# sloisel/MultiGridBarrier.jl

Hardware: AMD Instinct MI355X
Metric: Newton iters/sec + wall-clock to converge, 2D P2 p-Laplace L=9 (higher is better)
Workload: dtype f64

## Files before the change

include/mgbhip.h:

```cpp
#ifndef MGBHIP_H
#define MGBHIP_H

#include <stdint.h>

#ifdef __cplusplus
extern "C" {
#endif

#define MGBHIP_OK 0
#define MGBHIP_ERR_INVALID 1
#define MGBHIP_ERR_HIP 2
#define MGBHIP_ERR_NOT_SPD 3
#define MGBHIP_ERR_NONFINITE 4
#define MGBHIP_ERR_CONVERGENCE 5

#define MGBHIP_MAX_PIECES 4
#define MGBHIP_MAX_IDX 10
#define MGBHIP_MAX_LIN 4
#define MGBHIP_MAX_ND 13
#define MGBHIP_MAX_NU 4
#define MGBHIP_MAX_OPS 8

#define MGBHIP_KIND_EP 1
#define MGBHIP_KIND_LINEAR 2
// ... 116 lines not shown

int mgbhip_mgb_core(mgbhip_problem* prob, double* z , const double* c ,
                    const mgbhip_options* opt, mgbhip_core_result* res);
int mgbhip_matched_t(mgbhip_problem* prob, const double* z, const double* c, double t_default,
                     double* t_out);
void mgbhip_default_options(mgbhip_options* opt, int64_t n_nodes);

typedef struct mgbhip_vec mgbhip_vec;
int mgbhip_vec_alloc(mgbhip_ctx* ctx, int64_t len, mgbhip_vec** out);
int mgbhip_vec_free(mgbhip_vec* v);
int64_t mgbhip_vec_len(const mgbhip_vec* v);
int mgbhip_vec_upload(mgbhip_vec* v, const double* host, int64_t len);
int mgbhip_vec_download(const mgbhip_vec* v, double* host, int64_t len);
int mgbhip_vec_fill(mgbhip_vec* v, double value);
int mgbhip_vec_copy(mgbhip_vec* dst, const mgbhip_vec* src);
int mgbhip_vec_axpy(double alpha, const mgbhip_vec* x, mgbhip_vec* y);
int mgbhip_vec_scale(double alpha, mgbhip_vec* x);
int mgbhip_vec_dot(const mgbhip_vec* a, const mgbhip_vec* b, double* out);
int mgbhip_vec_norm(const mgbhip_vec* a, double* out);
int mgbhip_vec_isfinite(const mgbhip_vec* a, int32_t* all_finite);
int mgbhip_f0_d(mgbhip_problem* prob, int32_t level, const mgbhip_vec* s, const mgbhip_vec* c,
                const mgbhip_vec* z0, double* value);
int mgbhip_f1_d(mgbhip_problem* prob, int32_t level, const mgbhip_vec* s, const mgbhip_vec* c,
                const mgbhip_vec* z0, mgbhip_vec* grad);
int mgbhip_f2_d(mgbhip_problem* prob, int32_t level, const mgbhip_vec* s, const mgbhip_vec* c,
                const mgbhip_vec* z0);
int mgbhip_solve_d(mgbhip_problem* prob, int32_t level, const mgbhip_vec* g, mgbhip_vec* x);
int mgbhip_prolong_add(mgbhip_problem* prob, int32_t level, const mgbhip_vec* s, mgbhip_vec* z);

int mgbhip_stage_ms(mgbhip_problem* prob, const char* stage, double* total_ms, int64_t* launches);
int mgbhip_reset_stage_timers(mgbhip_problem* prob, int enable);
int mgbhip_solver_stats(mgbhip_problem* prob, int32_t level, double* out8);
int mgbhip_solver_chain(mgbhip_problem* prob, int32_t level, double* out8);
enum { MGBHIP_PROJ_NONE = 0, MGBHIP_PROJ_LOOP = 1, MGBHIP_PROJ_STAGED = 2, MGBHIP_PROJ_MFMA = 3, MGBHIP_PROJ_ACCUMULATE = 4 };
int mgbhip_level_plan(mgbhip_problem* prob, int32_t level, int32_t* out16);

#define MGBHIP_INTERP_FEM1D 1
#define MGBHIP_INTERP_QK 2
#define MGBHIP_INTERP_P1 3
#define MGBHIP_INTERP_P2 4
#define MGBHIP_INTERP_SPECTRAL1D 5
#define MGBHIP_INTERP_SPECTRAL2D 6
int mgbhip_interpolate(mgbhip_ctx* ctx, int32_t family, int32_t d, int32_t k, int32_t p, int64_t N,
                       const double* x, const double* table, int32_t ncomp, const double* z, int64_t M,
                       const double* pts, double* out, int32_t* elem);
int mgbhip_interpolate_grad(mgbhip_ctx* ctx, int32_t family, int32_t d, int32_t k, int32_t p, int64_t N,
                            const double* x, const double* table, int32_t ncomp, const double* z, int64_t M,
                            const double* pts, double* out ,
                            double* grad , int32_t* elem );

typedef struct mgbhip_locator mgbhip_locator;
int mgbhip_locator_create(mgbhip_ctx* ctx, int32_t family, int32_t d, int32_t k, int32_t p, int64_t N,
                          const double* x, const double* table, int64_t M, const double* pts,
                          mgbhip_locator** out);
int mgbhip_locator_elements(const mgbhip_locator* loc, int32_t* elem );
int mgbhip_locator_evaluate(mgbhip_locator* loc, int32_t ncomp, const double* z ,
                            double* out ,
                            double* grad );
int mgbhip_locator_destroy(mgbhip_locator* loc);

typedef struct mgbhip_contour mgbhip_contour;
int mgbhip_contour_create(mgbhip_ctx* ctx, int32_t family, int32_t d, int32_t k, int32_t p, int64_t N,
                          const double* x, const double* table, int32_t nfield , const double* fields,
                          int32_t nlevels, const double* levels, int32_t refine,
                          mgbhip_contour** out, int64_t* nsimplices);
int mgbhip_contour_fetch(const mgbhip_contour* c, double* points, int32_t* level, int32_t* element,
                         double* carried );
// ... 35 lines not shown
```

multigridbarrier.jl_amd/csrc/kernels.hip:

```cpp
#include <hip/hip_runtime.h>

#include <algorithm>
#include <mutex>

#include "kernels.hpp"
#include "dense.hpp"

namespace mgbhip {

namespace {

template <int CTRL>
__device__ __forceinline__ double dpp_mov_f64(double v) {
    const long long b = __double_as_longlong(v);
    const int lo = __builtin_amdgcn_mov_dpp((int)(b & 0xffffffffll), CTRL, 0xF, 0xF, true);
    const int hi = __builtin_amdgcn_mov_dpp((int)(b >> 32), CTRL, 0xF, 0xF, true);
    return __longlong_as_double(((long long)hi << 32) | (unsigned int)lo);
}
__device__ __forceinline__ double z_at(const ElemParams& P, int64_t i) {
    double v = P.z0[i];
    if (P.zsel) {
        const int32_t c = P.zsel[i];
        if (c >= 0) v += P.zx ? __builtin_fma(-P.zalpha, P.zx[c], P.zs[c]) : P.zs[c];
        if (P.zout) P.zout[i] = v;
// ... 419 lines not shown
                                } else if (idk) {
                                    val += Yt[i] * OP(k2, i, j);
                                } else if (idk2) {
                                    val += OP(k, j, i) * Yt[j];
                                } else {
                                    double acc = 0.0;
                                    for (int rr = 0; rr < p; ++rr) acc += OP(k, rr, i) * Yt[rr] * OP(k2, rr, j);
                                    val += acc;
                                }
                            }
                        }
                        out[i] = val;
                    }
                }
        }
        return;
    }
}

struct SigRuntime {
    static constexpr bool rt = true;
    static __device__ __forceinline__ constexpr int state(int) { return 0; }
    static __device__ __forceinline__ constexpr int stage(int) { return 0; }
    static __device__ __forceinline__ constexpr int mask() { return 0; }
};
template <int NY>
struct SigDefault {
    static constexpr bool rt = false;
    static __device__ __forceinline__ constexpr int state(int k) { return k == NY - 1 ? 1 : 0; }
    static __device__ __forceinline__ constexpr int stage(int k) { return (k == 0 || k == NY - 1) ? -1 : k - 1; }
    static __device__ __forceinline__ constexpr int mask() { return ((1 << NY) - 1) & ~1; }
};

template <int NY, int P, class Sig, bool CONDENSE = false>
__global__ __launch_bounds__(256) void elem_f2_fast(const ElemParams Pm) {
    constexpr int G = (P <= 2) ? 2 : (P <= 4) ? 4 : (P <= 8) ? 8 : (P <= 16) ? 16 : (P <= 32) ? 32 : 64;
    constexpr int EPB = 256 / G;
    constexpr int PP = P * P;
    constexpr int NT = NY * (NY + 1) / 2;
    extern __shared__ double sh[];
    const int tid = threadIdx.x;
    const int el = tid / G;
    const int r = tid % G;
    const int nu = Sig::rt ? Pm.nu : 2;
    auto DST = [&](int k) -> int { return Sig::rt ? Pm.D_state[k] : Sig::state(k); };
    auto DSG = [&](int k) -> int { return Sig::rt ? Pm.D_stage[k] : Sig::stage(k); };
    const int ymask = Sig::rt ? Pm.ymask : Sig::mask();
    const int64_t e0 = (int64_t)blockIdx.x * EPB;
    const int64_t e = e0 + el;
    const bool active = (e < Pm.N) && (r < P);
    const int64_t n = Pm.n;
    const int64_t node = e * P + r;

    double* zl = sh;
    double* opL = zl + 256 * nu;
    double* YL = opL + (size_t)Pm.nstage * EPB * PP;

    double zr[MGBHIP_MAX_NU];
#pragma unroll
    for (int a = 0; a < MGBHIP_MAX_NU; ++a) zr[a] = (active && a < nu) ? z_at(Pm, (int64_t)a * n + node) : 0.0;
    {
        int64_t lim = (Pm.N - e0) * PP;
        if (lim > (int64_t)EPB * PP) lim = (int64_t)EPB * PP;
        constexpr int NIT = (EPB * PP + 255) / 256;
        for (int o = 0; o < Pm.nstage; ++o) {
            const double* src = Pm.stage_ptr[o] + e0 * PP;
            double* dst = opL + (size_t)o * EPB * PP;
// ... 20 lines not shown
    auto OP = [&](int k, int rr, int cc) -> double { return opE[(size_t)DSG(k) * EPB * PP + cc * P + rr]; };

    double y[NY];
#pragma unroll
    for (int k = 0; k < NY; ++k) {
        double v = 0.0;
        if (active) {
            const double* za = zl + (el * nu + DST(k)) * G;
            if (DSG(k) < 0) v = za[r];
            else {
#pragma unroll
                for (int cc = 0; cc < P; ++cc) v += OP(k, r, cc) * za[cc];
            }
        }
        y[k] = v;
    }
    if (active) {
        double F, g[NY], H[NY * NY];
        cone_eval<NY, 2>(Pm.cone, node, n, y, F, g, H);
        const double bwv = Pm.bw ? Pm.bw[node] : 0.0;
#pragma unroll
        for (int k = 0; k < NY; ++k)
#pragma unroll
            for (int k2 = k; k2 < NY; ++k2) {
                const double h = H[k * NY + k2];
                YL[((size_t)el * NT + (k * NY - (k * (k - 1)) / 2 + (k2 - k))) * G + r] =
                    Pm.bw ? ((bwv == 0.0) ? 0.0 : bwv * h) : Pm.invn * h;
            }
    }
    __syncthreads();
    const int j = r;
    const double* Ye = YL + (size_t)el * NT * G;
    int blk = 0;
    double cblk[CONDENSE ? 3 : 1][P];
#pragma unroll
    for (int a = 0; a < nu; ++a)
#pragma unroll
        for (int b = a; b < nu; ++b, ++blk) {
            const bool dblk = CONDENSE ? (blk == 2) : ((Pm.diag_mask >> blk) & 1);
            double* dst = CONDENSE ? &cblk[blk < 3 ? blk : 0][0]
                                   : Pm.out_hel + Pm.blk_off[blk] + (dblk ? (e * P + j) : (e * P + j) * (int64_t)P);
            bool b_all_id = true;
#pragma unroll
            for (int k2 = 0; k2 < NY; ++k2)
                if (DST(k2) == b && ((ymask >> k2) & 1) && DSG(k2) >= 0) b_all_id = false;
            if (active && b_all_id) {
                double Cd[NY];
#pragma unroll
                for (int k = 0; k < NY; ++k) {
                    double acc = 0.0;
                    if (DST(k) == a && ((ymask >> k) & 1)) {
#pragma unroll
                        for (int k2 = 0; k2 < NY; ++k2) {
                            if (DST(k2) != b || !((ymask >> k2) & 1)) continue;
                            const int t = (k <= k2) ? (k * NY - (k * (k - 1)) / 2 + (k2 - k))
                                                    : (k2 * NY - (k2 * (k2 - 1)) / 2 + (k - k2));
                            acc += Ye[t * G + j];
                        }
                    }
                    Cd[k] = acc;
                }
                if (dblk) {
                    double val = 0.0;
#pragma unroll
                    for (int k = 0; k < NY; ++k)
                        if (DST(k) == a && ((ymask >> k) & 1)) val += Cd[k];
                    dst[0] = val;
                } else {
#pragma unroll
                    for (int i = 0; i < P; ++i) {
                        double val = 0.0;
#pragma unroll
                        for (int k = 0; k < NY; ++k) {
// ... 129 lines not shown
                    if (rr > j) S[at(rr, j)] = 0.0;
                S[at(P, j)] = usc[PB] * inv;
#pragma unroll
                for (int i = 0; i < PB; ++i)
                    if (pos[i] != 15) S[at(pos[i], j)] = usc[i] * inv;
                S[at(m - 1, j)] = beta * inv;
                if (j == PB) {
                    S[at(P, P)] = d7;
#pragma unroll
                    for (int i = 0; i < PB; ++i)
                        if (pos[i] != 15) S[at(pos[i], P)] = xc[i] * inv7;
                    S[at(m - 1, P)] = bb * inv7;
                    S[at(m - 1, m - 1)] = corner - bb * bb * inv7;
                } else if (pos[j] != 15) {
#pragma unroll
                    for (int i = 0; i < PB; ++i)
                        if (pos[i] != 15 && pos[i] >= pos[j]) S[at(pos[i], pos[j])] = up[i] - xc[i] * f;
                    S[at(m - 1, pos[j])] = bj - bb * f;
                }
            }
            if (pk) {
                __builtin_amdgcn_fence(__ATOMIC_RELEASE, "wavefront");
                __builtin_amdgcn_wave_barrier();
                __builtin_amdgcn_fence(__ATOMIC_ACQUIRE, "wavefront");
                if (e < Pm.N) {
                    const LeafDesc l2 = Pm.leaf_desc[e];
                    const int mm = (int)(l2.packed & 15u);
                    double* dstF = Pm.leaf_arena + l2.F_off;
                    for (int t = r; t < mm * (mm + 1) / 2; t += G) dstF[t] = S[t];
                }
            }
        }
        if (bad) atomicOr(Pm.leaf_status, 1);
    }
}

template <int NY, int P, class Sig>
__global__ __launch_bounds__(256) void elem_f01_fast(const ElemParams Pm) {
    constexpr int G = (P <= 2) ? 2 : (P <= 4) ? 4 : (P <= 8) ? 8 : (P <= 16) ? 16 : (P <= 32) ? 32 : 64;
    constexpr int EPB = 256 / G;
    constexpr int PP = P * P;
    extern __shared__ double sh[];
    const int tid = threadIdx.x;
    const int el = tid / G;
    const int r = tid % G;
    const int nu = Sig::rt ? Pm.nu : 2;
    auto DST = [&](int k) -> int { return Sig::rt ? Pm.D_state[k] : Sig::state(k); };
    auto DSG = [&](int k) -> int { return Sig::rt ? Pm.D_stage[k] : Sig::stage(k); };
    const int64_t e0 = (int64_t)blockIdx.x * EPB;
    const int64_t e = e0 + el;
    const bool active = (e < Pm.N) && (r < P);
    const int64_t n = Pm.n;
    const int64_t node = e * P + r;

    double* zl = sh;
    double* opL = zl + 256 * nu;
    double* YL = opL + (size_t)Pm.nstage * EPB * PP;
    {
        int64_t lim = (Pm.N - e0) * PP;
        if (lim > (int64_t)EPB * PP) lim = (int64_t)EPB * PP;
        constexpr int NIT = (EPB * PP + 255) / 256;
        for (int o = 0; o < Pm.nstage; ++o) {
            const double* src = Pm.stage_ptr[o] + e0 * PP;
            double* dst = opL + (size_t)o * EPB * PP;
            double v[NIT];
#pragma unroll
// ... 924 lines not shown
        (void)hipFuncSetAttribute((const void*)elem_f2_fast<NY, PN, SigDefault<NY>>, hipFuncAttributeMaxDynamicSharedMemorySize, 160 * 1024);
        (void)hipGetLastError();
        return true;
    }();
    (void)attr;
    if (is_default_signature<NY>(P))
        hipLaunchKernelGGL((elem_f2_fast<NY, PN, SigDefault<NY>>), dim3((unsigned)elem_grid(PN, P.N)), dim3(256), lds, st, P);
    else
        hipLaunchKernelGGL((elem_f2_fast<NY, PN, SigRuntime>), dim3((unsigned)elem_grid(PN, P.N)), dim3(256), lds, st, P);
    return true;
}

bool launch_elem_f2_condense(const ElemParams& P, hipStream_t st) {
    constexpr int NY = 4, PN = 7;
    if (P.wide || P.nD != NY || P.p != PN || P.nu != 2 || P.nstage != 2 || !is_default_signature<NY>(P)) return false;
    for (int k = 0; k < NY; ++k)
        if (P.D_stage[k] == -2) return false;
    MGB_REQUIRE(P.leaf_desc && P.leaf_arena && P.leaf_g && P.leaf_status, "condensing f2: leaf arguments missing");
    const int G = elem_group(PN);
    const int EPB = 256 / G;
    const size_t lds = (256 * (size_t)P.nu + (size_t)P.nstage * EPB * PN * PN + (size_t)EPB * (NY * (NY + 1) / 2) * G) * sizeof(double);
    static bool attr = [] {
        (void)hipFuncSetAttribute((const void*)elem_f2_fast<NY, PN, SigDefault<NY>, true>, hipFuncAttributeMaxDynamicSharedMemorySize, 160 * 1024);
        (void)hipGetLastError();
        return true;
    }();
    (void)attr;
    hipLaunchKernelGGL((elem_f2_fast<NY, PN, SigDefault<NY>, true>), dim3((unsigned)elem_grid(PN, P.N)), dim3(256), lds, st, P);
    MGB_HIP_CHECK(hipGetLastError());
    return true;
}

template <int NY, int PN>
static bool try_f01_fast(const ElemParams& P, hipStream_t st) {
    if (P.nD != NY || P.p != PN) return false;
    for (int k = 0; k < NY; ++k)
        if (P.D_stage[k] == -2) return false;
    const int G = elem_group(PN);
    const int EPB = 256 / G;
    size_t lds = (256 * (size_t)P.nu + (size_t)P.nstage * EPB * PN * PN + (size_t)EPB * NY * G) * sizeof(double);
    if (lds < 256 * sizeof(double)) lds = 256 * sizeof(double);
    if (lds > 160 * 1024) return false;
    static bool attr = [] {
        (void)hipFuncSetAttribute((const void*)elem_f01_fast<NY, PN, SigRuntime>, hipFuncAttributeMaxDynamicSharedMemorySize, 160 * 1024);
        (void)hipFuncSetAttribute((const void*)elem_f01_fast<NY, PN, SigDefault<NY>>, hipFuncAttributeMaxDynamicSharedMemorySize, 160 * 1024);
        (void)hipGetLastError();
        return true;
    }();
    (void)attr;
    if (is_default_signature<NY>(P))
        hipLaunchKernelGGL((elem_f01_fast<NY, PN, SigDefault<NY>>), dim3((unsigned)elem_grid(PN, P.N)), dim3(256), lds, st, P);
    else
        hipLaunchKernelGGL((elem_f01_fast<NY, PN, SigRuntime>), dim3((unsigned)elem_grid(PN, P.N)), dim3(256), lds, st, P);
    return true;
}

size_t wide_lds_bytes(int p, int nu, int nD, int nstage, int mode) {
    const int G = elem_group(p);
    const int threads = (mode == MODE_F2) ? WIDE_F2_THREADS : 256;
    const int EPB = threads / G;
    size_t d = (size_t)threads * nu + (size_t)nstage * EPB * p * p;
    if (mode == MODE_F1 || mode == MODE_F01) d += (size_t)threads * nD;
    if (mode == MODE_F2) d += (size_t)threads * (nD * (nD + 1) / 2);
    if (d < 256) d = 256;
    return d * sizeof(double);
}
// ... 326 lines not shown
void launch_panel_accumulate(const PanelParams& P, const int32_t* ecols, int32_t m, int32_t nstream, int32_t nsplit,
                             int32_t chunk, int32_t ctmax, double* partial, double* H, hipStream_t st) {
    if (m == 0) return;
    const size_t lds = ((size_t)chunk + panel_stage_doubles(P.p, P.nu, ctmax)) * sizeof(double);
    MGB_REQUIRE(lds <= PANEL_ACC_LDS_MAX, "coarse-level accumulator + panels exceed the LDS budget");
    MGB_REQUIRE(panel_accumulate_fits(P.p, P.nu, ctmax), "coarse-level panels exceed the register staging of the accumulation kernel");
    static std::once_flag once;
    std::call_once(once, [] {
        (void)hipFuncSetAttribute((const void*)panel_accumulate_kernel, hipFuncAttributeMaxDynamicSharedMemorySize,
                                  (int)PANEL_ACC_LDS_MAX);
        (void)hipGetLastError();
    });
    hipLaunchKernelGGL(panel_accumulate_kernel, dim3((unsigned)nstream, (unsigned)nsplit), dim3(256), lds, st, P, ecols, m,
                       ctmax, chunk, partial);
    hipLaunchKernelGGL(accumulate_reduce_kernel, dim3((unsigned)(((int64_t)m * m + 255) / 256)), dim3(256), 0, st, m,
                       nstream, partial, H);
    MGB_HIP_CHECK(hipGetLastError());
}

void launch_panel_project_staged(const PanelParams& P, int32_t ctmax, hipStream_t st) {
    if (P.N == 0) return;
    const size_t lds = panel_accumulate_lds(P.p, P.nu, ctmax);
    MGB_REQUIRE(lds <= PANEL_ACC_LDS_MAX, "coarse-level panels too wide for the staged projection kernel");
    static std::once_flag once;
    std::call_once(once, [] {
        (void)hipFuncSetAttribute((const void*)panel_project_staged_kernel, hipFuncAttributeMaxDynamicSharedMemorySize,
                                  (int)PANEL_ACC_LDS_MAX);
        (void)hipGetLastError();
    });
    hipLaunchKernelGGL(panel_project_staged_kernel, dim3((unsigned)((P.N + 3) / 4)), dim3(256), lds, st, P, ctmax);
    MGB_HIP_CHECK(hipGetLastError());
}

bool launch_panel_project_mfma(const PanelParams& P, hipStream_t st) {
    if (P.N == 0) return true;
    if (P.nu > MGBHIP_MAX_NU || P.p > 64) return false;
    const int ctpad = P.nu * pp_round_up(P.cmax, 16);
    const PanelMfmaLayout Y = panel_mfma_layout(P.p, P.nu, ctpad);
    const size_t lds = (size_t)Y.total * sizeof(double);
    static const bool off = [] { const char* e = getenv("MGBHIP_NO_MFMA_PROJECT"); return e && e[0] == '1'; }();
    if (off || lds > 64 * 1024 || ctpad < 48) return false;
    static std::once_flag once;
    std::call_once(once, [] {
        (void)hipFuncSetAttribute((const void*)panel_project_mfma_kernel, hipFuncAttributeMaxDynamicSharedMemorySize, 64 * 1024);
        (void)hipGetLastError();
    });
    hipLaunchKernelGGL(panel_project_mfma_kernel, dim3((unsigned)P.N), dim3(256), lds, st, P, ctpad);
    MGB_HIP_CHECK(hipGetLastError());
    return true;
}

void launch_invert_lists(const int32_t* cidx, int64_t total, int32_t* spos, hipStream_t st) {
    if (total <= 0) return;
    hipLaunchKernelGGL(invert_lists_kernel, dim3((unsigned)((total + 255) / 256)), dim3(256), 0, st, cidx, total, spos);
    MGB_HIP_CHECK(hipGetLastError());
}

void launch_panel_project(const PanelParams& P, hipStream_t st) {
    if (P.N == 0) return;
    const size_t lds = (size_t)4 * P.p * P.cmax * sizeof(double);
    static const bool big_lds = hipFuncSetAttribute((const void*)panel_project_kernel,
                                                    hipFuncAttributeMaxDynamicSharedMemorySize, 144 * 1024) == hipSuccess;
    if (!big_lds) (void)hipGetLastError();
    MGB_REQUIRE(lds <= (big_lds ? 144 : 64) * 1024, "coarse-level panels too wide for the projection kernel");
    hipLaunchKernelGGL(panel_project_kernel, dim3((unsigned)((P.N + 3) / 4)), dim3(256), lds, st, P);
    MGB_HIP_CHECK(hipGetLastError());
}

}
```

multigridbarrier.jl_amd/csrc/kernels.hpp:

```cpp
#pragma once
#include "common.hpp"
#include "cone.hpp"

namespace mgbhip {

enum ElemMode { MODE_F0 = 0, MODE_F1 = 1, MODE_F2 = 2, MODE_NODE_F = 3, MODE_NODE_SLACK = 4,
                MODE_F01 = 5 };

struct LeafDesc {
    int64_t F_off;
    int32_t interior;
    uint32_t packed;
};

struct ElemParams {
    int32_t p, nu, nD, nstage;
    int32_t ymask;
    int64_t N, n;
    const double* ops[MGBHIP_MAX_OPS];
    const double* stage_ptr[MGBHIP_MAX_OPS];
    int32_t D_state[MGBHIP_MAX_ND];
    int32_t D_op[MGBHIP_MAX_ND];
    int32_t D_stage[MGBHIP_MAX_ND];
    const double* w;
    const double* c;
    const double* z0;
    const double* bw;
    double invn;
    ConeDev cone;
    double* out_partial;
    double* out_ret;
    double* out_hel;
    double* out_F;
    double* out_Dz;
    int32_t diag_mask;
    int64_t blk_off[MGBHIP_MAX_NU * (MGBHIP_MAX_NU + 1) / 2];
    double* dn_Dz;
    double* dn_Y;
    const LeafDesc* leaf_desc;
    double* leaf_arena;
    const double* leaf_g;
    int64_t leaf_slack0;
    int32_t* leaf_status;
    int32_t leaf_packed;
    const int32_t* zsel;
    const double* zs;
    double* zout;
    const double* zx;
    double zalpha;
    int32_t wide;
};
static_assert(sizeof(ElemParams) <= 4096 - 64, "ElemParams must stay well inside the kernel argument limit");

bool launch_elem_f2_condense(const ElemParams& P, hipStream_t st);

inline int hel_blocks(int nu) { return nu * (nu + 1) / 2; }
inline int hel_block_index(int a, int b, int nu) { return a * nu - a * (a - 1) / 2 + (b - a); }
inline int64_t hel_layout(int nu, int64_t N, int p, int diag_mask, int64_t* off) {
    int64_t total = 0;
    for (int blk = 0; blk < hel_blocks(nu); ++blk) {
        off[blk] = total;
        total += ((diag_mask >> blk) & 1) ? N * p : N * (int64_t)p * p;
    }
    return total;
}

int elem_group(int p);
constexpr int WIDE_F2_THREADS = 128;
size_t wide_lds_bytes(int p, int nu, int nD, int nstage, int mode);
int64_t elem_grid(int p, int64_t N);
size_t elem_lds_bytes(const ElemParams& P, int mode);
void launch_elem(const ElemParams& P, int mode, hipStream_t st);

void launch_reduce_partials(const double* partials, int64_t count, double* out, hipStream_t st);
void launch_vec_stats(const double* v, int64_t n, double* scratch, double* stats, hipStream_t st, const double* mask = nullptr,
                      const int32_t* ints = nullptr, int nints = 0);
void launch_dir_stats(const double* v, const double* g, int64_t n, double* scratch, double* stats3, hipStream_t st,
                      const double* mask = nullptr, const int32_t* ints = nullptr, int nints = 0);
void launch_dot(const double* a, const double* b, int64_t n, double* scratch, double* out, hipStream_t st, const double* mask = nullptr);
void launch_restrict_trial(int64_t rows, const int32_t* ptr, const int32_t* col, const double* val, const double* ret, double* g,
                            double* scratch, const double* x, const double* nn, double s, double* xn, int32_t* moved, int32_t stamp,
                            hipStream_t st);
void launch_publish(const double* src, int n, double* host_block, int host_lo, double seq, hipStream_t st);
void launch_dir_finish(const double* v, const double* g, int64_t n, double* scratch, double* scal, int32_t* status2, double* host,
                       hipStream_t st, const double* mask = nullptr, double seq = 0.0);
void launch_trial_finish(const double* g, int64_t n, double* scratch, const double* f0_partials, int64_t f0_count, double* scal,
                         int32_t* moved, double* host, hipStream_t st, const double* mask = nullptr, double seq = 0.0,
// ... 5 lines not shown
void launch_csr_matvec(int64_t rows, const int32_t* ptr, const int32_t* col, const double* val,
                       const double* x, double* y, bool add, bool long_rows, hipStream_t st);
int csr_chunks(int64_t max_row_len);
void launch_csr_matvec_chunked(int64_t rows, const int32_t* ptr, const int32_t* col, const double* val,
                               const double* x, double* y, double* scratch, int nchunk, hipStream_t st);
void launch_prolong(int64_t rows, const int32_t* ptr, const int32_t* col, const double* val, const double* s,
                    const double* z0, double* zfull, hipStream_t st);
void launch_step(const double* x, const double* n, double s, double* xn, int64_t len, int32_t* moved, int32_t stamp,
                 hipStream_t st);
void launch_scale_copy(const double* src, double alpha, double* dst, int64_t len, hipStream_t st);
void launch_border_tail(const double* g, double* tail, int64_t m, hipStream_t st);
void launch_axpy(double alpha, const double* x, double* y, int64_t len, hipStream_t st);
void launch_fill(double value, double* y, int64_t len, hipStream_t st);

void launch_gather_shared(int64_t nshared, const int32_t* sh_q, const int32_t* cptr, const int32_t* cidx, const double* slab,
                          double* out, hipStream_t st);
void launch_gather_assemble(int64_t nnz, const int32_t* cptr, const int32_t* cidx, const double* slab,
                            double* Hval, bool long_lists, hipStream_t st, int32_t chunk = 0, int32_t nchunk = 0,
                            double* part = nullptr, const int32_t* qmap = nullptr, int64_t nq = 0);

struct PanelParams {
    int32_t p, nu;
    int64_t N;
    const int32_t* ecol_ptr;
    const double* panels;
    const int32_t* eoff;
    const double* hel;
    double* slab;
    int32_t cmax;
    int32_t upper_only;
    const int32_t* spos;
};
bool launch_panel_project_mfma(const PanelParams& P, hipStream_t st);
void launch_invert_lists(const int32_t* cidx, int64_t total, int32_t* spos, hipStream_t st);
void launch_panel_project(const PanelParams& P, hipStream_t st);
constexpr size_t PANEL_ACC_LDS_MAX = 144 * 1024;
size_t panel_accumulate_lds(int p, int nu, int ctmax);
size_t panel_stage_doubles(int p, int nu, int ctmax);
bool panel_accumulate_fits(int p, int nu, int ctmax);
void launch_panel_accumulate(const PanelParams& P, const int32_t* ecols, int32_t m, int32_t nstream, int32_t nsplit,
                             int32_t chunk, int32_t ctmax, double* partial, double* H, hipStream_t st);
void launch_panel_project_staged(const PanelParams& P, int32_t ctmax, hipStream_t st);

}
```

multigridbarrier.jl_amd/csrc/problem.cpp:

```cpp
#include "problem.hpp"
#include "plan_device.hpp"
#include "dense.hpp"

#include <algorithm>
#include <chrono>
#include <cmath>
#include <cstdio>
#include <atomic>
#include <exception>
#include <cstdlib>
#include <string>
#include <thread>
#include <cstring>
#include <numeric>

using namespace mgbhip;

static constexpr int64_t ACC_MAX_M = 384;



static void upload_csr(const mgbhip_csr& R, Level& L, hipStream_t st) {
    MGB_REQUIRE(R.rows >= 0 && R.cols >= 0 && R.rowptr && (R.rowptr[R.rows] == 0 || (R.colidx && R.values)),
                "bad prolongation CSR");
// ... 813 lines not shown
}

void mgbhip_problem::eval_f2(int level, const double* d_s, const double* d_zz, const double* d_cc, bool materialize,
                             const double* rhs) {
    ensure_plan(level);
    hipStream_t st = stream();
    Level& L = levels[level];
    int E_ymask = 0;
    if (L.condense && !materialize && rhs != nullptr && L.selection && L.direct && !dense) {
        StageScope sc(ctx->timers, level + 1 == (int)levels.size() ? "f2" : "f2_coarse");
        ElemParams E = base_params(level, d_s, d_zz, d_cc);
        E.leaf_desc = L.solver.leaf_desc();
        E.leaf_arena = L.solver.arena();
        E.leaf_g = rhs;
        E.leaf_slack0 = L.m - n;
        E.leaf_status = L.solver.leaf_status();
        E.leaf_packed = L.solver.leaves_packed() ? 1 : 0;
        if (!L.solver.leaf_flag_zero()) MGB_HIP_CHECK(hipMemsetAsync(E.leaf_status, 0, sizeof(int32_t), st));
        L.solver.leaf_flag_used();
        if (launch_elem_f2_condense(E, st)) {
            L.have_H = true;
            L.H_in_slab = true;
            L.H_condensed = true;
            L.condensed_rhs = rhs;
            hel_level = level;
            L.factored = false;
            cnt.f2++;
            return;
        }
        zf_stamp = -1;
    }
    L.H_condensed = false;
    L.proj_kernel = MGBHIP_PROJ_NONE;
    {
        StageScope sc(ctx->timers, level + 1 == (int)levels.size() ? "f2" : "f2_coarse");
        ElemParams E = base_params(level, d_s, d_zz, d_cc);
        E_ymask = E.ymask;
        E.diag_mask = (L.selection && !dense) ? diag_mask_sel : 0;
        hel_layout(nu, N, p, E.diag_mask, E.blk_off);
        launch_elem(E, MODE_F2, st);
    }
    {
        StageScope sc(ctx->timers, level + 1 == (int)levels.size() ? "assemble" : "assemble_coarse");
        if (dense) {
            int klo = nD, khi = -1;
            for (int k = 0; k < nD; ++k)
                if ((E_ymask >> k) & 1) { klo = std::min(klo, k); khi = std::max(khi, k); }
            const int64_t ld = (int64_t)nD * n;
            if (khi < klo) {
                MGB_HIP_CHECK(hipMemsetAsync(L.Hval.p, 0, sizeof(double) * (size_t)L.nnz, st));
            } else {
                launch_dense_weight(nD, klo, khi, n, L.m, ld, L.denseDR.p, d_dnY.p, L.denseW.p, st);
                launch_dense_gemm_tn((int)L.m, (int)L.m, (int)((khi - klo + 1) * n), L.denseDR.p + (int64_t)klo * n, ld,
                                     nullptr, L.denseW.p + (int64_t)klo * n, ld, L.Hval.p, L.m, false, true, st);
            }
        } else if (L.selection && L.direct && !materialize) {
            launch_gather_shared(L.nshared, L.sh_q.p, L.cptr.p, L.cidx.p, d_hel.p, d_hel.p + hel_cap, st);
        } else if (L.selection) {
            launch_gather_assemble(L.nnz, L.cptr.p, L.cidx.p, d_hel.p, L.Hval.p, L.long_lists, st, L.gather_chunk, L.gather_nchunk, L.gather_part.p);
        } else {
            PanelParams PP;
            PP.p = p; PP.nu = nu; PP.N = N;
            PP.ecol_ptr = L.ecol_ptr.p; PP.panels = L.panels.p; PP.eoff = L.eoff.p;
            PP.hel = d_hel.p; PP.slab = L.slab.p; PP.cmax = L.cmax; PP.spos = nullptr;
            static const bool full_h = [] { const char* e = getenv("MGBHIP_FULL_COARSE_H"); return e && e[0] == '1'; }();
            const bool upper = !materialize && rhs != nullptr && L.nup > 0 && !L.acc && !full_h;
            PP.upper_only = upper ? 1 : 0;
            if (L.acc) {
                L.proj_kernel = MGBHIP_PROJ_ACCUMULATE;
                launch_panel_accumulate(PP, L.ecols.p, (int32_t)L.m, L.acc_waves, L.acc_split, L.acc_chunk, L.acc_ctmax,
                                        L.acc_copies.p, L.Hval.p, st);
            } else {
                PP.spos = L.sorted_slab ? L.spos.p : nullptr;
                if (launch_panel_project_mfma(PP, st)) {
                    L.proj_kernel = MGBHIP_PROJ_MFMA;
                } else if (panel_accumulate_lds(p, nu, L.acc_ctmax) <= 40 * 1024) {
                    L.proj_kernel = MGBHIP_PROJ_STAGED;
                    launch_panel_project_staged(PP, L.acc_ctmax, st);
                } else {
                    L.proj_kernel = MGBHIP_PROJ_LOOP;
                    launch_panel_project(PP, st);
                }
                launch_gather_assemble(L.nnz, L.cptr.p, L.sorted_slab ? nullptr : L.cidx.p, L.slab.p, L.Hval.p, L.long_lists, st, L.gather_chunk,
                                       L.gather_nchunk, L.gather_part.p, upper ? L.upq.p : nullptr, upper ? L.nup : 0);
            }
        }
    }
    L.have_H = true;
    L.H_in_slab = L.selection && L.direct && !materialize && !dense;
    hel_level = L.H_in_slab ? level : -1;
    L.factored = false;
    cnt.f2++;
}

void mgbhip_problem::wait_results(double seq) {
    static const bool poll = [] { const char* e = getenv("MGBHIP_NO_POLL"); return !(e && e[0] == '1'); }();
    hipStream_t st = stream();
    if (poll && seq != 0.0) {
        volatile const double* stamp = pin.d + 15;
        const auto t0 = std::chrono::steady_clock::now();
        for (int spins = 0;; ++spins) {
            if (__atomic_load_n(reinterpret_cast<const volatile uint64_t*>(stamp), __ATOMIC_ACQUIRE) ==
                *reinterpret_cast<const uint64_t*>(&seq))
                return;
            if ((spins & 1023) == 1023 &&
                std::chrono::duration<double>(std::chrono::steady_clock::now() - t0).count() > 1e-3)
                break;
// ... 175 lines not shown
```

multigridbarrier.jl_amd/device.py:

```python
from __future__ import annotations

import ctypes as C
import os
import weakref
from typing import List, Optional

import numpy as np
import scipy.sparse as sp

from .blockmatrices import BlockColumn, BlockDiag
from .convex import KIND_EP, KIND_LINEAR, Convex
from .multigrid import AMG
from .problem import MGBProblem

MAX_PIECES, MAX_IDX, MAX_ND, MAX_NU, MAX_OPS = 4, 10, 13, 4, 8
MAX_LIN = 4
OK, ERR_INVALID, ERR_HIP, ERR_NOT_SPD, ERR_NONFINITE, ERR_CONVERGENCE = range(6)


class Device:
    """reference: src/device.jl:18"""


class CPUDevice(Device):
# ... 556 lines not shown
                    factorizations=int(r.factorizations), failure_code=int(r.failure_code), k=int(r.k))
        return status, z, diag

    def matched_t(self, z, c, t_default: float) -> float:
        z = _f64(z)
        c = np.asfortranarray(c, dtype=np.float64)
        out = C.c_double()
        _check(self.lib, self.lib.mgbhip_matched_t(self.handle, _ptr(z), _ptr(c), float(t_default), C.cast(C.byref(out), _dp)))
        return out.value

    def reset_stage_timers(self, enable: bool = True):
        _check(self.lib, self.lib.mgbhip_reset_stage_timers(self.handle, 1 if enable else 0))

    def stage_ms(self, stage: str):
        ms, cnt = C.c_double(), C.c_int64()
        _check(self.lib, self.lib.mgbhip_stage_ms(self.handle, stage.encode(), C.cast(C.byref(ms), _dp), C.byref(cnt)))
        return ms.value, cnt.value

    def solver_stats(self, level: int) -> dict:
        out = np.zeros(8)
        _check(self.lib, self.lib.mgbhip_solver_stats(self.handle, level, _ptr(out)))
        keys = ("fronts", "max_front", "arena_doubles", "factor_flops", "peeled", "tree_levels", "nnz", "unknowns")
        return dict(zip(keys, out.tolist()))

    def solver_chain(self, level: int) -> dict:
        out = np.zeros(8)
        _check(self.lib, self.lib.mgbhip_solver_chain(self.handle, level, _ptr(out)))
        keys = ("pivot_blocks_on_critical_path", "large_front_tree_levels", "launches_per_factorization",
                "launches_per_backward_sweep", "arena_doubles", "factor_flops", "extra_trailing_doubles", "reserved")
        return dict(zip(keys, out.tolist()))

    PLAN_KEYS = ("R_unit", "R_long", "T_long", "T_chunks", "selection", "acc", "acc_split", "long_lists", "gather_chunk",
                 "gather_nchunk", "projection", "max_row", "max_col", "cmax", "mean_list", "planned")
    PROJECTION = ("none", "loop", "staged", "mfma", "accumulate")

    def level_plan(self, level: int) -> dict:
        out = (C.c_int32 * 16)()
        _check(self.lib, self.lib.mgbhip_level_plan(self.handle, level, out))
        d = dict(zip(self.PLAN_KEYS, (int(v) for v in out)))
        d["projection"] = self.PROJECTION[d["projection"]]
        d["direct"] = bool(d["selection"] & 2)
        d["selection"] = bool(d["selection"] & 1)
        for k in ("R_unit", "R_long", "T_long", "acc", "long_lists", "planned"):
            d[k] = bool(d[k])
        return d

    def close(self):
        if self.handle:
            self.lib.mgbhip_problem_destroy(self.handle)
            self.handle = None

    def __del__(self):
        try:
            self.close()
        except Exception:
            pass


def dense_as_block(M: AMG) -> AMG:
    if isinstance(M.D_fine[0], BlockColumn):
        return M
    n = M.w.size
    geom = M.geometry
    ops = {k: BlockDiag(np.asarray(v, dtype=np.float64).reshape(n, n, 1)) for k, v in geom.operators.items()}
    from dataclasses import replace
    g2 = replace(geom, operators=ops)
    nu = len(M.state_names)
# ... 49 lines not shown
```

Before: 674.3.

## Fuse coarse-level panel projection into the element Hessian f2 kernel

Adds a PROJECT variant of elem_f2_fast that keeps each element's 2x2-block Hessian in LDS and immediately projects it through the prolongation panels (P^T H P), writing directly into the coarse slab. It is used when the MFMA projection does not apply, in place of a separate f2 kernel plus a staged projection kernel. This removes the global write and read of the per-element Hessian and one launch per coarse level. In exchange it adds LDS pressure and wave-level serial work per element inside the f2 kernel, and it only covers a few hardcoded (NY,P) instantiations.

```diff
diff --git a/include/mgbhip.h b/include/mgbhip.h
--- a/include/mgbhip.h
+++ b/include/mgbhip.h
@@ -172,7 +172,8 @@
 int mgbhip_reset_stage_timers(mgbhip_problem* prob, int enable);
 int mgbhip_solver_stats(mgbhip_problem* prob, int32_t level, double* out8);
 int mgbhip_solver_chain(mgbhip_problem* prob, int32_t level, double* out8);
-enum { MGBHIP_PROJ_NONE = 0, MGBHIP_PROJ_LOOP = 1, MGBHIP_PROJ_STAGED = 2, MGBHIP_PROJ_MFMA = 3, MGBHIP_PROJ_ACCUMULATE = 4 };
+enum { MGBHIP_PROJ_NONE = 0, MGBHIP_PROJ_LOOP = 1, MGBHIP_PROJ_STAGED = 2, MGBHIP_PROJ_MFMA = 3, MGBHIP_PROJ_ACCUMULATE = 4,
+       MGBHIP_PROJ_FUSED = 5  };
 int mgbhip_level_plan(mgbhip_problem* prob, int32_t level, int32_t* out16);
 
 #define MGBHIP_INTERP_FEM1D 1
diff --git a/multigridbarrier.jl_amd/csrc/kernels.hip b/multigridbarrier.jl_amd/csrc/kernels.hip
--- a/multigridbarrier.jl_amd/csrc/kernels.hip
+++ b/multigridbarrier.jl_amd/csrc/kernels.hip
@@ -475,7 +475,7 @@
     static __device__ __forceinline__ constexpr int mask() { return ((1 << NY) - 1) & ~1; }
 };
 
-template <int NY, int P, class Sig, bool CONDENSE = false>
+template <int NY, int P, class Sig, bool CONDENSE = false, bool PROJECT = false>
 __global__ __launch_bounds__(256) void elem_f2_fast(const ElemParams Pm) {
     constexpr int G = (P <= 2) ? 2 : (P <= 4) ? 4 : (P <= 8) ? 8 : (P <= 16) ? 16 : (P <= 32) ? 32 : 64;
     constexpr int EPB = 256 / G;
@@ -562,13 +562,13 @@
     const int j = r;
     const double* Ye = YL + (size_t)el * NT * G;
     int blk = 0;
-    double cblk[CONDENSE ? 3 : 1][P];
+    double cblk[(CONDENSE || PROJECT) ? 3 : 1][P];
 #pragma unroll
     for (int a = 0; a < nu; ++a)
 #pragma unroll
         for (int b = a; b < nu; ++b, ++blk) {
-            const bool dblk = CONDENSE ? (blk == 2) : ((Pm.diag_mask >> blk) & 1);
-            double* dst = CONDENSE ? &cblk[blk < 3 ? blk : 0][0]
+            const bool dblk = CONDENSE ? (blk == 2) : PROJECT ? false : ((Pm.diag_mask >> blk) & 1);
+            double* dst = (CONDENSE || PROJECT) ? &cblk[blk < 3 ? blk : 0][0]
                                    : Pm.out_hel + Pm.blk_off[blk] + (dblk ? (e * P + j) : (e * P + j) * (int64_t)P);
             bool b_all_id = true;
 #pragma unroll
@@ -764,6 +764,96 @@
             }
         }
         if (bad) atomicOr(Pm.leaf_status, 1);
+    }
+    if constexpr (PROJECT) {
+        static_assert(!Sig::rt && !CONDENSE && P <= 8, "projection: default two-state signature only");
+        constexpr int NBLK = 3, EPW = 64 / G, NROW = 2 * P, NPF = ELEM_PROJECT_PREFETCH;
+        const int lane = tid & 63;
+        const int wave = __builtin_amdgcn_readfirstlane(tid >> 6);
+        const int ctmax = Pm.pj_ctmax;
+        __syncthreads();
+        if (active) {
+            double* Hc = sh + (size_t)el * (NBLK * PP) + P * j;
+#pragma unroll
+            for (int b3 = 0; b3 < NBLK; ++b3)
+#pragma unroll
+                for (int i = 0; i < P; ++i) Hc[b3 * PP + i] = cblk[b3][i];
+        }
+        double* Pl = sh + (size_t)EPB * (NBLK * PP) + (size_t)wave * (3 * P) * ctmax;
+        double* Tl = Pl + (size_t)P * ctmax;
+        int32_t nct = 0, nc0 = 0, neo = 0;
+        double rP[NPF];
+        auto prefetch = [&](int64_t ee) {
+            const int32_t base = Pm.pj_ecol_ptr[ee * 2];
+            nc0 = Pm.pj_ecol_ptr[ee * 2 + 1] - base;
+            nct = Pm.pj_ecol_ptr[ee * 2 + 2] - base;
+            neo = Pm.pj_eoff[ee];
+            const double* pan = Pm.pj_panels + (int64_t)P * base;
+#pragma unroll
+            for (int u = 0; u < NPF; ++u) {
+                const int t = lane + 64 * u;
+                rP[u] = t < P * nct ? pan[t] : 0.0;
+            }
+        };
+        const int64_t ew0 = e0 + (int64_t)wave * EPW;
+        if (ew0 < Pm.N) prefetch(ew0);
+        for (int k = 0; k < EPW; ++k) {
+            const int64_t ee = ew0 + k;
+            if (ee >= Pm.N) break;
+            const int ct = nct, c0 = nc0;
+            const int64_t eo = neo;
+            __builtin_amdgcn_fence(__ATOMIC_RELEASE, "wavefront");
+            __builtin_amdgcn_wave_barrier();
+            __builtin_amdgcn_fence(__ATOMIC_ACQUIRE, "wavefront");
+#pragma unroll
+            for (int u = 0; u < NPF; ++u) {
+                const int t = lane + 64 * u;
+                if (t < P * ct) Pl[t] = rP[u];
+            }
+            if (k + 1 < EPW && ee + 1 < Pm.N) prefetch(ee + 1);
+            __builtin_amdgcn_fence(__ATOMIC_RELEASE, "wavefront");
+            __builtin_amdgcn_wave_barrier();
+            __builtin_amdgcn_fence(__ATOMIC_ACQUIRE, "wavefront");
+            const double* Hl = sh + (size_t)(wave * EPW + k) * (NBLK * PP);
+            for (int t = lane; t < NROW * ct; t += 64) {
+                const int jc = t / NROW, row = t - jc * NROW;
+                const int a = row / P, rr = row - a * P;
+                const int b = jc >= c0 ? 1 : 0;
+                const bool tr = a > b;
+                const int blk = tr ? (b * 2 - (b * (b - 1)) / 2 + (a - b)) : (a * 2 - (a * (a - 1)) / 2 + (b - a));
+                const double* Hb = Hl + (size_t)blk * PP;
+                double acc = 0.0;
+#pragma unroll
+                for (int ss = 0; ss < P; ++ss) acc += (tr ? Hb[ss + P * rr] : Hb[rr + P * ss]) * Pl[ss + P * jc];
+                Tl[row + NROW * jc] = acc;
+            }
+            __builtin_amdgcn_fence(__ATOMIC_RELEASE, "wavefront");
+            __builtin_amdgcn_wave_barrier();
+            __builtin_amdgcn_fence(__ATOMIC_ACQUIRE, "wavefront");
+            if (Pm.pj_upper) {
+                for (int t = lane; t < ct * (ct + 1) / 2; t += 64) {
+                    int jc = (int)((sqrtf(8.0f * (float)t + 1.0f) - 1.0f) * 0.5f);
+                    while ((jc + 1) * (jc + 2) / 2 <= t) ++jc;
+                    while (jc * (jc + 1) / 2 > t) --jc;
+                    const int i = t - jc * (jc + 1) / 2;
+                    const int a = i >= c0 ? 1 : 0;
+                    double acc = 0.0;
+#pragma unroll
+                    for (int rr = 0; rr < P; ++rr) acc += Pl[rr + P * i] * Tl[(a * P + rr) + NROW * jc];
+                    const int64_t o = eo + i + ct * jc;
+                    Pm.pj_slab[Pm.pj_spos ? Pm.pj_spos[o] : o] = acc;
+                }
+            } else {
+                for (int t = lane; t < ct * ct; t += 64) {
+                    const int jc = t / ct, i = t - jc * ct;
+                    const int a = i >= c0 ? 1 : 0;
+                    double acc = 0.0;
+#pragma unroll
+                    for (int rr = 0; rr < P; ++rr) acc += Pl[rr + P * i] * Tl[(a * P + rr) + NROW * jc];
+                    Pm.pj_slab[Pm.pj_spos ? Pm.pj_spos[eo + t] : eo + t] = acc;
+                }
+            }
+        }
     }
 }
 
@@ -1754,6 +1844,38 @@
 }
 
 template <int NY, int PN>
+static bool try_f2_project(const ElemParams& P, hipStream_t st) {
+    if (P.nD != NY || P.p != PN || !is_default_signature<NY>(P)) return false;
+    for (int k = 0; k < NY; ++k)
+        if (P.D_stage[k] == -2) return false;
+    const int G = elem_group(PN);
+    const int EPB = 256 / G;
+    if (PN * P.pj_ctmax > 64 * ELEM_PROJECT_PREFETCH) return false;
+    const size_t eval = 256 * (size_t)P.nu + (size_t)P.nstage * EPB * PN * PN + (size_t)EPB * (NY * (NY + 1) / 2) * G;
+    const size_t proj = (size_t)EPB * 3 * PN * PN + (size_t)4 * 3 * PN * P.pj_ctmax;
+    const size_t lds = std::max(eval, proj) * sizeof(double);
+    if (lds > 64 * 1024) return false;
+    static bool attr = [] {
+        (void)hipFuncSetAttribute((const void*)elem_f2_fast<NY, PN, SigDefault<NY>, false, true>, hipFuncAttributeMaxDynamicSharedMemorySize, 64 * 1024);
+        (void)hipGetLastError();
+        return true;
+    }();
+    (void)attr;
+    hipLaunchKernelGGL((elem_f2_fast<NY, PN, SigDefault<NY>, false, true>), dim3((unsigned)elem_grid(PN, P.N)), dim3(256), lds, st, P);
+    return true;
+}
+
+bool launch_elem_f2_project(const ElemParams& P, hipStream_t st) {
+    if (P.wide || P.p > 8 || P.nu != 2 || P.diag_mask != 0 || P.N == 0) return false;
+    MGB_REQUIRE(P.pj_ecol_ptr && P.pj_panels && P.pj_eoff && P.pj_slab && P.pj_ctmax > 0, "projecting f2: panel arguments missing");
+    if (try_f2_project<4, 7>(P, st) || try_f2_project<3, 2>(P, st) || try_f2_project<4, 6>(P, st) || try_f2_project<6, 2>(P, st)) {
+        MGB_HIP_CHECK(hipGetLastError());
+        return true;
+    }
+    return false;
+}
+
+template <int NY, int PN>
 static bool try_f01_fast(const ElemParams& P, hipStream_t st) {
     if (P.nD != NY || P.p != PN) return false;
     for (int k = 0; k < NY; ++k)
@@ -2146,14 +2268,22 @@
     MGB_HIP_CHECK(hipGetLastError());
 }
 
-bool launch_panel_project_mfma(const PanelParams& P, hipStream_t st) {
+bool panel_project_mfma_applies(const PanelParams& P) {
     if (P.N == 0) return true;
     if (P.nu > MGBHIP_MAX_NU || P.p > 64) return false;
     const int ctpad = P.nu * pp_round_up(P.cmax, 16);
     const PanelMfmaLayout Y = panel_mfma_layout(P.p, P.nu, ctpad);
     const size_t lds = (size_t)Y.total * sizeof(double);
     static const bool off = [] { const char* e = getenv("MGBHIP_NO_MFMA_PROJECT"); return e && e[0] == '1'; }();
-    if (off || lds > 64 * 1024 || ctpad < 48) return false;
+    return !(off || lds > 64 * 1024 || ctpad < 48);
+}
+
+bool launch_panel_project_mfma(const PanelParams& P, hipStream_t st) {
+    if (P.N == 0) return true;
+    if (!panel_project_mfma_applies(P)) return false;
+    const int ctpad = P.nu * pp_round_up(P.cmax, 16);
+    const PanelMfmaLayout Y = panel_mfma_layout(P.p, P.nu, ctpad);
+    const size_t lds = (size_t)Y.total * sizeof(double);
     static std::once_flag once;
     std::call_once(once, [] {
         (void)hipFuncSetAttribute((const void*)panel_project_mfma_kernel, hipFuncAttributeMaxDynamicSharedMemorySize, 64 * 1024);
diff --git a/multigridbarrier.jl_amd/csrc/kernels.hpp b/multigridbarrier.jl_amd/csrc/kernels.hpp
--- a/multigridbarrier.jl_amd/csrc/kernels.hpp
+++ b/multigridbarrier.jl_amd/csrc/kernels.hpp
@@ -49,10 +49,20 @@
     const double* zx;
     double zalpha;
     int32_t wide;
+    const int32_t* pj_ecol_ptr;
+    const double* pj_panels;
+    const int32_t* pj_eoff;
+    double* pj_slab;
+    const int32_t* pj_spos;
+    int32_t pj_ctmax;
+    int32_t pj_upper;
 };
 static_assert(sizeof(ElemParams) <= 4096 - 64, "ElemParams must stay well inside the kernel argument limit");
 
 bool launch_elem_f2_condense(const ElemParams& P, hipStream_t st);
+
+constexpr int ELEM_PROJECT_PREFETCH = 2;
+bool launch_elem_f2_project(const ElemParams& P, hipStream_t st);
 
 inline int hel_blocks(int nu) { return nu * (nu + 1) / 2; }
 inline int hel_block_index(int a, int b, int nu) { return a * nu - a * (a - 1) / 2 + (b - a); }
@@ -124,6 +134,7 @@
     const int32_t* spos;
 };
 bool launch_panel_project_mfma(const PanelParams& P, hipStream_t st);
+bool panel_project_mfma_applies(const PanelParams& P);
 void launch_invert_lists(const int32_t* cidx, int64_t total, int32_t* spos, hipStream_t st);
 void launch_panel_project(const PanelParams& P, hipStream_t st);
 constexpr size_t PANEL_ACC_LDS_MAX = 144 * 1024;
diff --git a/multigridbarrier.jl_amd/csrc/problem.cpp b/multigridbarrier.jl_amd/csrc/problem.cpp
--- a/multigridbarrier.jl_amd/csrc/problem.cpp
+++ b/multigridbarrier.jl_amd/csrc/problem.cpp
@@ -869,13 +869,33 @@
     }
     L.H_condensed = false;
     L.proj_kernel = MGBHIP_PROJ_NONE;
+    PanelParams PP;
+    std::memset(&PP, 0, sizeof(PP));
+    bool upper = false, fused = false;
+    if (!dense && !L.selection) {
+        PP.p = p; PP.nu = nu; PP.N = N;
+        PP.ecol_ptr = L.ecol_ptr.p; PP.panels = L.panels.p; PP.eoff = L.eoff.p;
+        PP.hel = d_hel.p; PP.slab = L.slab.p; PP.cmax = L.cmax;
+        static const bool full_h = [] { const char* e = getenv("MGBHIP_FULL_COARSE_H"); return e && e[0] == '1'; }();
+        upper = !materialize && rhs != nullptr && L.nup > 0 && !L.acc && !full_h;
+        PP.upper_only = upper ? 1 : 0;
+        PP.spos = (!L.acc && L.sorted_slab) ? L.spos.p : nullptr;
+    }
     {
         StageScope sc(ctx->timers, level + 1 == (int)levels.size() ? "f2" : "f2_coarse");
         ElemParams E = base_params(level, d_s, d_zz, d_cc);
         E_ymask = E.ymask;
         E.diag_mask = (L.selection && !dense) ? diag_mask_sel : 0;
         hel_layout(nu, N, p, E.diag_mask, E.blk_off);
-        launch_elem(E, MODE_F2, st);
+        static const bool no_fused = [] { const char* e = getenv("MGBHIP_NO_FUSED_PROJECT"); return e && e[0] == '1'; }();
+        if (!no_fused && !materialize && rhs != nullptr && !dense && !L.selection && !L.acc && !wide && !sharded() && N > 0 &&
+            L.slab_doubles > 0 && !panel_project_mfma_applies(PP) && panel_accumulate_lds(p, nu, L.acc_ctmax) <= 40 * 1024) {
+            E.pj_ecol_ptr = PP.ecol_ptr; E.pj_panels = PP.panels; E.pj_eoff = PP.eoff; E.pj_slab = PP.slab; E.pj_spos = PP.spos;
+            E.pj_ctmax = L.acc_ctmax;
+            E.pj_upper = PP.upper_only;
+            fused = launch_elem_f2_project(E, st);
+        }
+        if (!fused) launch_elem(E, MODE_F2, st);
     }
     {
         StageScope sc(ctx->timers, level + 1 == (int)levels.size() ? "assemble" : "assemble_coarse");
@@ -896,20 +916,14 @@
         } else if (L.selection) {
             launch_gather_assemble(L.nnz, L.cptr.p, L.cidx.p, d_hel.p, L.Hval.p, L.long_lists, st, L.gather_chunk, L.gather_nchunk, L.gather_part.p);
         } else {
-            PanelParams PP;
-            PP.p = p; PP.nu = nu; PP.N = N;
-            PP.ecol_ptr = L.ecol_ptr.p; PP.panels = L.panels.p; PP.eoff = L.eoff.p;
-            PP.hel = d_hel.p; PP.slab = L.slab.p; PP.cmax = L.cmax; PP.spos = nullptr;
-            static const bool full_h = [] { const char* e = getenv("MGBHIP_FULL_COARSE_H"); return e && e[0] == '1'; }();
-            const bool upper = !materialize && rhs != nullptr && L.nup > 0 && !L.acc && !full_h;
-            PP.upper_only = upper ? 1 : 0;
             if (L.acc) {
                 L.proj_kernel = MGBHIP_PROJ_ACCUMULATE;
                 launch_panel_accumulate(PP, L.ecols.p, (int32_t)L.m, L.acc_waves, L.acc_split, L.acc_chunk, L.acc_ctmax,
                                         L.acc_copies.p, L.Hval.p, st);
             } else {
-                PP.spos = L.sorted_slab ? L.spos.p : nullptr;
-                if (launch_panel_project_mfma(PP, st)) {
+                if (fused) {
+                    L.proj_kernel = MGBHIP_PROJ_FUSED;
+                } else if (launch_panel_project_mfma(PP, st)) {
                     L.proj_kernel = MGBHIP_PROJ_MFMA;
                 } else if (panel_accumulate_lds(p, nu, L.acc_ctmax) <= 40 * 1024) {
                     L.proj_kernel = MGBHIP_PROJ_STAGED;
diff --git a/multigridbarrier.jl_amd/device.py b/multigridbarrier.jl_amd/device.py
--- a/multigridbarrier.jl_amd/device.py
+++ b/multigridbarrier.jl_amd/device.py
@@ -612,7 +612,7 @@
 
     PLAN_KEYS = ("R_unit", "R_long", "T_long", "T_chunks", "selection", "acc", "acc_split", "long_lists", "gather_chunk",
                  "gather_nchunk", "projection", "max_row", "max_col", "cmax", "mean_list", "planned")
-    PROJECTION = ("none", "loop", "staged", "mfma", "accumulate")
+    PROJECTION = ("none", "loop", "staged", "mfma", "accumulate", "fused")
 
     def level_plan(self, level: int) -> dict:
         out = (C.c_int32 * 16)()
```

Result: faster. 683.8, median of 6 (+1.4%).
